# jackBonadies/Guided-Attention

Hardware: NVIDIA B200
Metric: guided_images_per_s (higher is better)
Workload: dtype f16

## Files before the change

guided_attention_b200/_cabi.py:

```python
from __future__ import annotations

import ctypes as C
import os
import threading

_HERE = os.path.dirname(os.path.abspath(__file__))
LIB_PATH = os.path.join(_HERE, "csrc", "libguidedattn.so")

GA_OK = 0
GA_F32, GA_F16, GA_BF16 = 0, 1, 2
GA_IMPL_AUTO, GA_IMPL_SIMT, GA_IMPL_TCGEN05, GA_IMPL_TCGEN05_SINGLE, GA_IMPL_TCGEN05_PIPE = 0, 1, 2, 3, 4
GA_TOKEN_COOR, GA_TOKEN_BOX, GA_TOKEN_KEYWORD = 0, 1, 2
GA_MAX_ACC_SLICES, GA_MAX_TOKENS, GA_MAX_BOXES, GA_MAX_CTX = 32, 24, 32, 128
(GA_STAT_MAX, GA_STAT_SUM, GA_STAT_COL, GA_STAT_ROW, GA_STAT_INSIDE, GA_STAT_OUTSIDE, GA_STAT_SCALED,
 GA_STAT_UNSCALED, GA_STAT_HINGE_IN, GA_STAT_HINGE_OUT, GA_STAT_NINSIDE, GA_STAT_CENTER, GA_STAT_RAW_SUM,
 GA_STAT_RAW_COL, GA_STAT_RAW_ROW) = range(15)
GA_STATS = 16
GA_ABI_VERSION = 7
GA_STEP_CTL_BYTES, GA_STEP_COUNTER_BASE = 256, 19
(GA_STEP_N_EVAL, GA_STEP_N_UPDATE, GA_STEP_N_CFG, GA_STEP_N_REFINE, GA_STEP_N_ROUNDS, GA_STEP_N_RENOISE) = range(6)


class GaToken(C.Structure):
    _fields_ = [("column", C.c_int32), ("kind", C.c_int32), ("box", C.c_int32), ("group", C.c_int32),
# ... 10 lines not shown

class GaScoreBias(C.Structure):
    _fields_ = [("mask", C.c_void_p), ("mask_stride_bh", C.c_int64), ("mask_stride_n", C.c_int64),
                ("pww_masks", C.c_void_p), ("pww_coef", C.c_void_p), ("pww_smax", C.c_void_p),
                ("pww_count", C.c_int32), ("pww_column", C.c_int32 * GA_MAX_TOKENS)]


class GaStepPrograms(C.Structure):
    _fields_ = [(n, C.c_void_p) for n in ("eval", "update", "cfg", "advance", "renoise", "refine_update")]


class GaStepParams(C.Structure):
    _fields_ = [("thr_call", C.c_double), ("thr_cfg", C.c_double), ("thr_last", C.c_double),
                ("has_thr_call", C.c_int32), ("has_thr_cfg", C.c_int32), ("has_thr_last", C.c_int32),
                ("check", C.c_int32), ("update_cond", C.c_int32), ("recurse_ok", C.c_int32),
                ("renoise_ok", C.c_int32), ("recurse_steps", C.c_int32), ("max_refine", C.c_int32),
                ("timestep", C.c_int64), ("step_size", C.c_float), ("ddim", C.c_float * 4),
                ("renoise", C.c_float * 2)]


_vp, _i, _f, _i64 = C.c_void_p, C.c_int, C.c_float, C.c_int64
_bias = C.POINTER(GaScoreBias)

PROTOTYPES = {
    "ga_version": (_i, []),
    "ga_last_error": (C.c_char_p, []),
    "ga_device_supported": (_i, [_i]),
    "ga_cross_attn_fwd": (_i, [_vp, _vp, _vp, _vp, _vp, _vp, _i, _i, _i, _i, _i, _f, _i, _i, _vp]),
    "ga_cross_attn_bwd": (_i, [_vp, _vp, _vp, _vp, _vp, _vp, _i64, _i, _vp, _vp, _vp, _i, _i, _i, _i, _i, _f, _i, _i,
                                _vp]),
    "ga_attn_probs": (_i, [_vp, _vp, _vp, _i, _i, _i, _i, _i, _f, _i, _vp]),
    "ga_cross_attn_smax": (_i, [_vp, _vp, _vp, _bias, _i, _i, _i, _i, _i, _f, _i, _vp]),
    "ga_cross_attn_fwd_ex": (_i, [_vp, _vp, _vp, _vp, _vp, _vp, _bias, _i, _i, _i, _i, _i, _f, _i, _i, _vp]),
    "ga_cross_attn_bwd_ex": (_i, [_vp, _vp, _vp, _vp, _vp, _vp, _i64, _i, _vp, _vp, _vp, _bias, _vp, _i, _i, _i, _i, _i,
                                   _f, _i, _i, _vp]),
    "ga_attn_probs_ex": (_i, [_vp, _vp, _vp, _bias, _i, _i, _i, _i, _i, _f, _i, _vp]),
    "ga_self_attn_fwd": (_i, [_vp, _vp, _vp, _vp, _vp, _i, _i, _i, _i, _f, _i, _vp]),
    "ga_self_attn_bwd": (_i, [_vp, _vp, _vp, _vp, _vp, _vp, _vp, _vp, _vp, _vp, _i, _i, _i, _i, _f, _i, _vp]),
    "ga_rasterize_boxes": (_i, [C.POINTER(C.c_double), _i, _i, C.c_double, _vp, _vp]),
    "ga_guidance_tail_fwd": (_i, [C.POINTER(_vp), C.POINTER(C.c_int32), _i, C.POINTER(GaTailParams), C.POINTER(GaToken),
                                  _vp, _vp, _vp, _vp, _vp, _vp, _vp, _vp, _vp]),
    "ga_guidance_tail_bwd": (_i, [C.POINTER(GaTailParams), C.POINTER(GaToken), _vp, _vp, _vp, _vp, _vp, _vp, _vp, _vp,
                                  _vp, _vp, _i, _vp]),
    "ga_step_driver_create": (_i, [C.POINTER(_vp), C.POINTER(GaStepPrograms), _vp, _vp, _vp, _vp, _vp, _vp, _vp, _vp,
                                   C.POINTER(GaToken), _i, _i, _i, _vp, _vp, _vp, _vp]),
    "ga_step_driver_run": (_i, [_vp, C.POINTER(GaStepParams), _vp]),
    "ga_step_driver_set_params": (_i, [_vp, C.POINTER(GaStepParams), _vp]),
    "ga_step_driver_destroy": (_i, [_vp]),
    "ga_smooth_fwd": (_i, [_vp, _vp, _i, _i, C.POINTER(C.c_float), _vp]),
    "ga_smooth_bwd": (_i, [_vp, _vp, _i, _i, C.POINTER(C.c_float), _vp]),
    "ga_box_loss_fwd": (_i, [_vp, _vp, _vp, _i, _i, _vp, _vp]),
    "ga_box_loss_bwd": (_i, [_vp, _vp, _vp, _i, _i, _vp, _vp, _vp]),
    "ga_group_norm_ws_bytes": (_i64, [_i, _i, _i, _i]),
    "ga_group_norm_fwd": (_i, [_vp, _vp, _i64, _vp, _vp, _vp, _vp, _vp, _i, _i, _i, _i, _f, _i, _i, _vp]),
    "ga_group_norm_bwd": (_i, [_vp, _vp, _i64, _vp, _vp, _vp, _vp, _vp, _vp, _i, _i, _i, _i, _i, _i, _vp]),
    "ga_add_bias_residual": (_i, [_vp, _vp, _vp, _vp, _i64, _i, _i, _vp]),
    "ga_layer_norm_fwd": (_i, [_vp, _vp, _vp, _vp, _vp, _vp, _i64, _i, _f, _i, _vp]),
    "ga_geglu_fwd": (_i, [_vp, _vp, _i64, _i, _i, _vp]),
    "ga_geglu_bwd": (_i, [_vp, _vp, _vp, _i64, _i, _i, _vp]),
}

_lib = None
_lock = threading.Lock()


class GuidedAttnLibraryError(RuntimeError):
    pass


def load(path: str = None) -> C.CDLL:
    global _lib
    with _lock:
        if _lib is not None and path is None:
            return _lib
        p = path or os.environ.get("GA_LIB_PATH", LIB_PATH)
        if not os.path.isfile(p):
            raise GuidedAttnLibraryError(
                f"{p} not found: build it with `python -c 'import __graft_entry__ as g; g.build()'` "
                "(nvcc, sm_100a).  The guidance path has no CPU or PyTorch fallback.")
        lib = C.CDLL(p)
        for name, (res, args) in PROTOTYPES.items():
            fn = getattr(lib, name)
            fn.restype, fn.argtypes = res, args
        if lib.ga_version() != GA_ABI_VERSION:
            raise GuidedAttnLibraryError(f"ABI mismatch: library {lib.ga_version()} vs binding {GA_ABI_VERSION}")
        if path is None:
            _lib = lib
        return lib


def check(rc: int, what: str):
    if rc != GA_OK:
        msg = load().ga_last_error().decode("utf-8", "replace")
        raise GuidedAttnLibraryError(f"{what} failed ({rc}): {msg}")
```

guided_attention_b200/csrc/unet_ops.cu:

```cuda
#include "ga_common.cuh"
#include <stdlib.h>

namespace ga {
namespace gn {

constexpr int kThreads = 256;

struct Params {
  const void* x;
  const void* dy;
  const void* gamma;
  const void* beta;
  const void* shift;
  int64_t shift_stride;
  void* out;
  float* stats;
  float* ws;
  int n, hw, c, groups, cpg;
  int cs;
  int vs;
  int pl;
  int chunk;
  int P;
  float eps;
};

template <typename T> __device__ __forceinline__ void unpack8(const uint4& w, float* f) {
  const float2 a = Word<T>::unpack(w.x), b = Word<T>::unpack(w.y), c = Word<T>::unpack(w.z), d = Word<T>::unpack(w.w);
  f[0] = a.x; f[1] = a.y; f[2] = b.x; f[3] = b.y; f[4] = c.x; f[5] = c.y; f[6] = d.x; f[7] = d.y;
}
template <typename T> __device__ __forceinline__ uint4 pack8(const float* f) {
  return make_uint4(Word<T>::pack(f[0], f[1]), Word<T>::pack(f[2], f[3]), Word<T>::pack(f[4], f[5]),
                    Word<T>::pack(f[6], f[7]));
}
__device__ __forceinline__ float sigmoidf_fast(float z) { return __fdividef(1.f, 1.f + __expf(-z)); }
__device__ __forceinline__ void pdl_wait() { asm volatile("griddepcontrol.wait;" ::: "memory"); }
__device__ __forceinline__ void pdl_launch_dependents() { asm volatile("griddepcontrol.launch_dependents;" ::: "memory"); }

struct Coord {
  int n, c0, pl, p0, p1;
  bool active;
  __device__ __forceinline__ void init(const Params& p) {
    const int tid = threadIdx.x;
    pl = tid / p.vs;
    const int v = tid - pl * p.vs;
    active = pl < p.pl;
    n = blockIdx.z;
    c0 = ((int)blockIdx.y * p.vs + v) * 8;
    p0 = (int)blockIdx.x * p.chunk;
    p1 = min(p0 + p.chunk, p.hw);
  }
};

template <typename T> __device__ __forceinline__ void load_shift(const Params& p, const Coord& t, float* sh) {
  if (p.shift != nullptr) {
    unpack8<T>(__ldg(reinterpret_cast<const uint4*>(reinterpret_cast<const T*>(p.shift) + (int64_t)t.n * p.shift_stride + t.c0)), sh);
  } else {
#pragma unroll
    for (int e = 0; e < 8; ++e) sh[e] = 0.f;
  }
}

__device__ __forceinline__ void group_partials(const Params& p, const Coord& t, const float* s, const float* q,
                                               float4* part, float& S, float& Q, int& g_out, bool& owner) {
  const int g0 = t.c0 / p.cpg;
  const int k = min(8, (g0 + 1) * p.cpg - t.c0);
  float sA = 0.f, qA = 0.f, sB = 0.f, qB = 0.f;
#pragma unroll
  for (int e = 0; e < 8; ++e) {
    if (e < k) { sA += s[e]; qA += q[e]; } else { sB += s[e]; qB += q[e]; }
  }
  part[threadIdx.x] = t.active ? make_float4(sA, qA, sB, qB) : make_float4(0.f, 0.f, 0.f, 0.f);
  __syncthreads();
  const int gps = p.groups / p.cs;
  const int sub = gps * 8 <= kThreads ? 8 : 1;
  const int gl = (int)threadIdx.x / sub, j = (int)threadIdx.x - gl * sub;
  const bool live = gl < gps;
  const int slice_c0 = (int)blockIdx.y * p.vs * 8;
  const int g = (int)blockIdx.y * gps + gl;
  S = 0.f; Q = 0.f;
  if (live) {
    const int v_lo = (g * p.cpg - slice_c0) >> 3, v_hi = ((g + 1) * p.cpg - 1 - slice_c0) >> 3;
    for (int l = j; l < p.pl; l += sub)
      for (int v = v_lo; v <= v_hi; ++v) {
        const float4 w = part[l * p.vs + v];
        if (slice_c0 + v * 8 >= g * p.cpg) { S += w.x; Q += w.y; } else { S += w.z; Q += w.w; }
      }
  }
  if (sub == 8) {
#pragma unroll
    for (int off = 4; off > 0; off >>= 1) {
      S += __shfl_down_sync(0xffffffffu, S, off, 8);
      Q += __shfl_down_sync(0xffffffffu, Q, off, 8);
    }
  }
  owner = live && j == 0;
  g_out = g;
}

constexpr int kMaxChunks = 128;
constexpr int kMaxSliceGroups = 32;
constexpr int kMergeLoads = 16;

__device__ __forceinline__ int merge_tpg(int gps) {
  int tpg = 8;
  while (tpg < 32 && tpg * 2 * gps <= kThreads) tpg *= 2;
  return tpg;
}

__device__ __forceinline__ void merge_stats(const Params& p, float2* sst) {
  pdl_wait();
  const int gps = p.groups / p.cs, n = blockIdx.z;
  const int tpg = merge_tpg(gps);
  const int gl = (int)threadIdx.x / tpg, j = (int)threadIdx.x - gl * tpg;
  const bool live = gl < gps;
  const int g = (int)blockIdx.y * gps + gl;
  float2 w[kMergeLoads];
#pragma unroll
  for (int i = 0; i < kMergeLoads; ++i) {
    const int ch = j + tpg * i;
    w[i] = (live && ch < p.P) ? __ldg(reinterpret_cast<const float2*>(p.ws) + ((int64_t)n * p.P + ch) * p.groups + g)
                              : make_float2(0.f, 0.f);
  }
  float cnt = 0.f, mean = 0.f, m2 = 0.f;
#pragma unroll
  for (int i = 0; i < kMergeLoads; ++i) {
    const int ch = j + tpg * i;
    if (live && ch < p.P) {
      const float cb = (float)((min((ch + 1) * p.chunk, p.hw) - ch * p.chunk) * p.cpg);
      const float tot = cnt + cb, delta = w[i].x - mean, f = __fdividef(cb, tot);
      mean = fmaf(delta, f, mean);
      m2 += w[i].y + delta * delta * cnt * f;
      cnt = tot;
    }
  }
#pragma unroll
  for (int off = 16; off > 0; off >>= 1) {
    if (off < tpg) {
      const float cb = __shfl_down_sync(0xffffffffu, cnt, off, 32);
      const float mb = __shfl_down_sync(0xffffffffu, mean, off, 32);
      const float qb = __shfl_down_sync(0xffffffffu, m2, off, 32);
      if (cb > 0.f && j + off < tpg) {
        const float tot = cnt + cb, delta = mb - mean, f = __fdividef(cb, tot);
        mean = fmaf(delta, f, mean);
        m2 += qb + delta * delta * cnt * f;
        cnt = tot;
// ... 184 lines not shown
template <typename T, bool kSilu>
__global__ void __launch_bounds__(kThreads) gn_bwd_apply_kernel(const Params p) {
  __shared__ float2 scf[kMaxSliceGroups];
  Coord t;
  t.init(p);
  merge_sums(p, scf);
  if (!t.active) return;
  float a[8], b[8], gr[8], r[8], mr[8], k1[8], k2[8];
  {
    float gm[8], bt[8];
    const int g_first = (int)blockIdx.y * (p.groups / p.cs);
    unpack8<T>(__ldg(reinterpret_cast<const uint4*>(reinterpret_cast<const T*>(p.gamma) + t.c0)), gm);
    unpack8<T>(__ldg(reinterpret_cast<const uint4*>(reinterpret_cast<const T*>(p.beta) + t.c0)), bt);
    float sh[8];
    load_shift<T>(p, t, sh);
#pragma unroll
    for (int e = 0; e < 8; ++e) {
      const int g = (t.c0 + e) / p.cpg;
      const float2 st = __ldg(reinterpret_cast<const float2*>(p.stats) + t.n * p.groups + g);
      const float2 cf = scf[g - g_first];
      const float mu = st.x - sh[e];
      r[e] = st.y;
      mr[e] = mu * st.y;
      a[e] = st.y * gm[e];
      b[e] = fmaf(-mu, a[e], bt[e]);
      gr[e] = gm[e] * st.y;
      k1[e] = cf.x * st.y;
      k2[e] = cf.y * st.y;
    }
  }
  const int64_t base = ((int64_t)t.n * p.hw) * p.c + t.c0;
  const uint4* xp = reinterpret_cast<const uint4*>(reinterpret_cast<const T*>(p.x) + base);
  const uint4* gp = reinterpret_cast<const uint4*>(reinterpret_cast<const T*>(p.dy) + base);
  uint4* op = reinterpret_cast<uint4*>(reinterpret_cast<T*>(p.out) + base);
  const int64_t stride = (int64_t)p.c / 8;
#pragma unroll 2
  for (int px = t.p0 + t.pl; px < t.p1; px += p.pl) {
    float f[8], d[8];
    unpack8<T>(__ldg(xp + px * stride), f);
    unpack8<T>(__ldg(gp + px * stride), d);
#pragma unroll
    for (int e = 0; e < 8; ++e) {
      float dz = d[e];
      if (kSilu) {
        const float z = fmaf(f[e], a[e], b[e]);
        const float sg = sigmoidf_fast(z);
        dz *= sg * fmaf(z, 1.f - sg, 1.f);
      }
      const float xh = fmaf(f[e], r[e], -mr[e]);
      f[e] = fmaf(dz, gr[e], -k1[e]) - xh * k2[e];
    }
    op[px * stride] = pack8<T>(f);
  }
}

static bool plan(Params& p, int n, int hw, int c, int groups) {
  if (n < 1 || hw < 1 || c < 8 || groups < 1 || c % groups != 0 || c % 8 != 0) return false;
  if ((int64_t)n * groups > (1 << 20)) return false;
  p.n = n; p.hw = hw; p.c = c; p.groups = groups; p.cpg = c / groups;
  const int V = c / 8;
  int cs = (V + kThreads - 1) / kThreads;
  while (cs <= groups && (groups % cs != 0 || V % cs != 0 || ((V / cs) * 8) % p.cpg != 0 || V / cs > kThreads)) ++cs;
  if (cs > groups) return false;
  p.cs = cs;
  p.vs = V / cs;
  p.pl = kThreads / p.vs;
  for (int v = 0; v < V; ++v)
    if ((v * 8 + 7) / p.cpg - (v * 8) / p.cpg > 1) return false;
  int chunk = (hw + 127) / 128;
  if (chunk < p.pl) chunk = p.pl;
  if (chunk > hw) chunk = hw;
  p.chunk = chunk;
  p.P = (hw + chunk - 1) / chunk;
  if (p.P > kMaxChunks || groups / cs > kMaxSliceGroups || n > 65535 || cs > 65535) return false;
  return true;
}

int64_t ws_bytes(int n, int hw, int c, int groups) {
  Params p;
  if (!plan(p, n, hw, c, groups)) return -1;
  return (int64_t)n * p.P * groups * 2 * (int64_t)sizeof(float);
}

static bool use_pdl() {
  static int v = -1;
  if (v < 0) {
    const char* e = getenv("GA_GN_PDL");
    v = (e != nullptr && e[0] == '0') ? 0 : 1;
  }
  return v == 1;
}

template <typename K>
static void launch_second(K kernel, const dim3& grid, const Params& p, cudaStream_t st) {
  cudaLaunchConfig_t cfg = {};
  cfg.gridDim = grid;
  cfg.blockDim = dim3(kThreads);
  cfg.dynamicSmemBytes = 0;
  cfg.stream = st;
  cudaLaunchAttribute attr[1];
  attr[0].id = cudaLaunchAttributeProgrammaticStreamSerialization;
  attr[0].val.programmaticStreamSerializationAllowed = 1;
  cfg.attrs = attr;
  cfg.numAttrs = use_pdl() ? 1 : 0;
  cudaLaunchKernelEx(&cfg, kernel, p);
}

template <typename T>
static void launch_fwd(const Params& p, bool silu, cudaStream_t st) {
  const dim3 grid(p.P, p.cs, p.n);
  gn_stats_kernel<T><<<grid, kThreads, 0, st>>>(p);
  if (silu) launch_second(gn_apply_kernel<T, true>, grid, p, st);
  else launch_second(gn_apply_kernel<T, false>, grid, p, st);
}
template <typename T>
static void launch_bwd(const Params& p, bool silu, cudaStream_t st) {
  const dim3 grid(p.P, p.cs, p.n);
  if (silu) {
    gn_bwd_sums_kernel<T, true><<<grid, kThreads, 0, st>>>(p);
    launch_second(gn_bwd_apply_kernel<T, true>, grid, p, st);
  } else {
    gn_bwd_sums_kernel<T, false><<<grid, kThreads, 0, st>>>(p);
    launch_second(gn_bwd_apply_kernel<T, false>, grid, p, st);
  }
}

int fwd(const void* x, const void* shift, int64_t shift_stride, const void* gamma, const void* beta, void* y, float* stats, float* ws, int n,
        int hw, int c, int groups, float eps, int silu, int dtype, cudaStream_t st) {
  Params p;
  if (!plan(p, n, hw, c, groups))
    return fail(GA_ERR_UNSUPPORTED, "group norm: shape n=%d hw=%d c=%d groups=%d is not supported", n, hw, c, groups);
  p.x = x; p.shift = shift; p.shift_stride = shift_stride; p.dy = nullptr; p.gamma = gamma; p.beta = beta; p.out = y; p.stats = stats; p.ws = ws;
  p.eps = eps;
  if (dtype == GA_F16) launch_fwd<__half>(p, silu != 0, st);
  else launch_fwd<__nv_bfloat16>(p, silu != 0, st);
  return check_launch("group_norm_fwd");
}

int bwd(const void* x, const void* shift, int64_t shift_stride, const void* dy, const void* gamma, const void* beta, const float* stats,
        void* dx, float* ws, int n, int hw, int c, int groups, int silu, int dtype, cudaStream_t st) {
  Params p;
  if (!plan(p, n, hw, c, groups))
    return fail(GA_ERR_UNSUPPORTED, "group norm: shape n=%d hw=%d c=%d groups=%d is not supported", n, hw, c, groups);
  p.x = x; p.shift = shift; p.shift_stride = shift_stride; p.dy = dy; p.gamma = gamma; p.beta = beta; p.out = dx; p.stats = const_cast<float*>(stats); p.ws = ws;
  p.eps = 0.f;
  if (dtype == GA_F16) launch_bwd<__half>(p, silu != 0, st);
  else launch_bwd<__nv_bfloat16>(p, silu != 0, st);
  return check_launch("group_norm_bwd");
}

template <typename T>
__global__ void __launch_bounds__(kThreads) add_bias_residual_kernel(const uint4* __restrict__ a, const uint4* __restrict__ b,
                                                                     const uint4* __restrict__ bias, uint4* __restrict__ out,
                                                                     int64_t n_vec, int vec_per_pixel) {
  for (int64_t i = (int64_t)blockIdx.x * kThreads + threadIdx.x; i < n_vec; i += (int64_t)gridDim.x * kThreads) {
    float fa[8], fb[8], fc[8];
    unpack8<T>(__ldg(a + i), fa);
    unpack8<T>(__ldg(bias + (int)(i % vec_per_pixel)), fc);
    if (b != nullptr) {
      unpack8<T>(__ldg(b + i), fb);
#pragma unroll
      for (int e = 0; e < 8; ++e) fa[e] += fb[e];
    }
#pragma unroll
    for (int e = 0; e < 8; ++e) fa[e] += fc[e];
    out[i] = pack8<T>(fa);
  }
}

int add_bias_residual(const void* a, const void* b, const void* bias, void* out, int64_t n_pixels, int c, int dtype,
                      cudaStream_t st) {
  const int64_t n_vec = n_pixels * (c / 8);
  if (n_vec == 0) return GA_OK;
  int64_t blocks = (n_vec + kThreads - 1) / kThreads;
  if (blocks > 148 * 8) blocks = 148 * 8;
  const uint4 *pa = static_cast<const uint4*>(a), *pb = static_cast<const uint4*>(b), *pc = static_cast<const uint4*>(bias);
  if (dtype == GA_F16)
    add_bias_residual_kernel<__half><<<(int)blocks, kThreads, 0, st>>>(pa, pb, pc, static_cast<uint4*>(out), n_vec, c / 8);
  else
    add_bias_residual_kernel<__nv_bfloat16><<<(int)blocks, kThreads, 0, st>>>(pa, pb, pc, static_cast<uint4*>(out), n_vec,
                                                                             c / 8);
  return check_launch("add_bias_residual");
}

__device__ __forceinline__ float gelu_f(float g) { return 0.5f * g * (1.f + erff(g * 0.70710678118654752f)); }
__device__ __forceinline__ float gelu_grad_f(float g) {
  return 0.5f * (1.f + erff(g * 0.70710678118654752f)) + g * 0.3989422804014327f * __expf(-0.5f * g * g);
}

template <typename T>
__global__ void __launch_bounds__(kThreads) geglu_fwd_kernel(const uint4* __restrict__ p, uint4* __restrict__ out,
                                                             int64_t n_vec, int vec_per_row) {
  for (int64_t i = (int64_t)blockIdx.x * kThreads + threadIdx.x; i < n_vec; i += (int64_t)gridDim.x * kThreads) {
    const int64_t r = i / vec_per_row;
    const int v = (int)(i - r * vec_per_row);
    float h[8], g[8];
    unpack8<T>(__ldg(p + r * 2 * vec_per_row + v), h);
    unpack8<T>(__ldg(p + r * 2 * vec_per_row + vec_per_row + v), g);
#pragma unroll
    for (int e = 0; e < 8; ++e) h[e] *= gelu_f(g[e]);
    out[i] = pack8<T>(h);
// ... 116 lines not shown
  GA_CHECK_ARG(x && gamma && beta && y && mean && rstd, "NULL operand");
  GA_CHECK_ARG(dtype == GA_F16 || dtype == GA_BF16, "layer norm: 16-bit activations only (dtype %d)", dtype);
  GA_CHECK_ARG(rows >= 0 && rows < ((int64_t)1 << 34) && channels >= 8 && channels % 8 == 0 &&
                   channels <= 32 * 8 * gn::kLnMaxVec,
               "layer norm: channels %d must be a multiple of 8 in [8, %d]", channels, 32 * 8 * gn::kLnMaxVec);
  GA_CHECK_ALIGN(x, 16, "x");
  GA_CHECK_ALIGN(y, 16, "y");
  GA_CHECK_ALIGN(gamma, 16, "gamma");
  GA_CHECK_ALIGN(beta, 16, "beta");
  return gn::layer_norm_fwd(x, gamma, beta, y, mean, rstd, rows, channels, eps, dtype, static_cast<cudaStream_t>(stream));
}

static int check_geglu_args(const void* p, const void* out, int64_t rows, int inner, int dtype) {
  GA_CHECK_ARG(p && out, "NULL operand");
  GA_CHECK_ARG(dtype == GA_F16 || dtype == GA_BF16, "geglu: 16-bit activations only (dtype %d)", dtype);
  GA_CHECK_ARG(rows >= 0 && inner >= 8 && inner % 8 == 0, "geglu: inner width %d must be a multiple of 8", inner);
  GA_CHECK_ALIGN(p, 16, "proj");
  GA_CHECK_ALIGN(out, 16, "output");
  return GA_OK;
}

extern "C" int ga_geglu_fwd(const void* proj, void* out, int64_t rows, int inner, int dtype, ga_stream_t stream) {
  int rc = check_geglu_args(proj, out, rows, inner, dtype);
  if (rc != GA_OK) return rc;
  return gn::geglu(proj, nullptr, out, rows, inner, dtype, false, static_cast<cudaStream_t>(stream));
}

extern "C" int ga_geglu_bwd(const void* proj, const void* d_out, void* d_proj, int64_t rows, int inner, int dtype,
                            ga_stream_t stream) {
  int rc = check_geglu_args(proj, d_proj, rows, inner, dtype);
  if (rc != GA_OK) return rc;
  GA_CHECK_ARG(d_out != nullptr, "NULL operand");
  GA_CHECK_ALIGN(d_out, 16, "d_out");
  return gn::geglu(proj, d_out, d_proj, rows, inner, dtype, true, static_cast<cudaStream_t>(stream));
}

extern "C" int ga_add_bias_residual(const void* a, const void* b, const void* bias, void* out, int64_t n_pixels,
                                    int channels, int dtype, ga_stream_t stream) {
  GA_CHECK_ARG(a && bias && out, "NULL operand");
  GA_CHECK_ARG(dtype == GA_F16 || dtype == GA_BF16, "add_bias_residual: 16-bit activations only (dtype %d)", dtype);
  GA_CHECK_ARG(n_pixels >= 0 && channels >= 8 && channels % 8 == 0, "add_bias_residual: channels %d must be a multiple of 8",
               channels);
  GA_CHECK_ALIGN(a, 16, "a");
  GA_CHECK_ALIGN(out, 16, "out");
  GA_CHECK_ALIGN(bias, 16, "bias");
  if (b != nullptr) GA_CHECK_ALIGN(b, 16, "b");
  return gn::add_bias_residual(a, b, bias, out, n_pixels, channels, dtype, static_cast<cudaStream_t>(stream));
}

extern "C" int64_t ga_group_norm_ws_bytes(int n, int hw, int channels, int groups) {
  return gn::ws_bytes(n, hw, channels, groups);
}

static int check_gn_args(const void* x, const void* gamma, const void* beta, const void* out, const void* stats,
                         const void* ws, int dtype) {
  GA_CHECK_ARG(x && gamma && beta && out && stats && ws, "NULL operand");
  GA_CHECK_ARG(dtype == GA_F16 || dtype == GA_BF16, "group norm: 16-bit activations only (dtype %d)", dtype);
  GA_CHECK_ALIGN(x, 16, "x");
  GA_CHECK_ALIGN(out, 16, "output");
  GA_CHECK_ALIGN(gamma, 16, "gamma");
  GA_CHECK_ALIGN(beta, 16, "beta");
  GA_CHECK_ALIGN(stats, 8, "stats");
  GA_CHECK_ALIGN(ws, 8, "ws");
  return GA_OK;
}

extern "C" int ga_group_norm_fwd(const void* x, const void* shift, int64_t shift_stride, const void* gamma, const void* beta, void* y,
                                 float* stats, float* ws, int n, int hw, int channels, int groups, float eps, int silu,
                                 int dtype, ga_stream_t stream) {
  int rc = check_gn_args(x, gamma, beta, y, stats, ws, dtype);
  if (rc != GA_OK) return rc;
  if (shift != nullptr) {
    GA_CHECK_ALIGN(shift, 16, "shift");
    GA_CHECK_ARG(shift_stride >= channels && shift_stride % 8 == 0, "shift_stride %lld must be a multiple of 8 >= channels",
                 (long long)shift_stride);
  }
  return gn::fwd(x, shift, shift_stride, gamma, beta, y, stats, ws, n, hw, channels, groups, eps, silu, dtype,
                 static_cast<cudaStream_t>(stream));
}

extern "C" int ga_group_norm_bwd(const void* x, const void* shift, int64_t shift_stride, const void* d_y, const void* gamma, const void* beta,
                                 const float* stats, void* d_x, float* ws, int n, int hw, int channels, int groups,
                                 int silu, int dtype, ga_stream_t stream) {
  int rc = check_gn_args(x, gamma, beta, d_x, stats, ws, dtype);
  if (rc != GA_OK) return rc;
  GA_CHECK_ARG(d_y != nullptr, "NULL operand");
  GA_CHECK_ALIGN(d_y, 16, "d_y");
  if (shift != nullptr) {
    GA_CHECK_ALIGN(shift, 16, "shift");
    GA_CHECK_ARG(shift_stride >= channels && shift_stride % 8 == 0, "shift_stride %lld must be a multiple of 8 >= channels",
                 (long long)shift_stride);
  }
  return gn::bwd(x, shift, shift_stride, d_y, gamma, beta, stats, d_x, ws, n, hw, channels, groups, silu, dtype,
                 static_cast<cudaStream_t>(stream));
}
```

guided_attention_b200/ops.py:

```python
from __future__ import annotations

import ctypes as C
import math
import os
from dataclasses import dataclass, field
from typing import List, Optional, Sequence

import numpy as np
import torch

from . import _cabi as abi

launch_counts = {}


def _count(name, n=1):
    launch_counts[name] = launch_counts.get(name, 0) + n


def total_launches() -> int:
    return sum(launch_counts.values())


def reset_launch_counts():
# ... 280 lines not shown
        ctx.save_for_backward(q.contiguous(), k.contiguous(), v.contiguous(), o, lse)
        ctx.meta = (heads, float(scale))
        return o

    @staticmethod
    def backward(ctx, d_o):
        q, k, v, o, lse = ctx.saved_tensors
        heads, scale = ctx.meta
        lib = abi.load()
        B, N, Cdim = q.shape
        d = Cdim // heads
        d_o = d_o.contiguous()
        d_q, d_k, d_v = torch.empty_like(q), torch.empty_like(k), torch.empty_like(v)
        dvec = torch.empty((B, heads, N), dtype=torch.float32, device=q.device)
        with torch.cuda.device(q.device), _span("self_attn_bwd", (B, heads, N, d, str(q.dtype)),
                                                self_attn_flops(B, heads, N, d, "bwd"), q.device):
            abi.check(lib.ga_self_attn_bwd(_ptr(q), _ptr(k), _ptr(v), _ptr(o), _ptr(lse), _ptr(d_o), _ptr(d_q),
                                           _ptr(d_k), _ptr(d_v), _ptr(dvec), B, heads, N, d, scale,
                                           _DTYPES[q.dtype], _stream(q)), "ga_self_attn_bwd")
        _count("self_attn_bwd", 2)
        return d_q, d_k, d_v, None, None


def self_attention(q, k, v, heads: int, scale: float):
    return _SelfAttnFn.apply(q, k, v, heads, scale)


def self_attention_supported(dtype, head_dim: int) -> bool:
    return dtype in (torch.float16, torch.bfloat16) and head_dim % 8 == 0 and 8 <= head_dim <= 160


def attention_probs(q, k, heads: int, scale: float, bias=None):
    _need_cuda(q, k)
    lib = abi.load()
    q, k = q.contiguous(), k.contiguous()
    B, N, Cdim = q.shape
    T = k.shape[1]
    p = torch.empty((B * heads, N, T), dtype=q.dtype, device=q.device)
    with torch.cuda.device(q.device):
        if bias is not None:
            if bias.has_pww and bias.smax is None:
                score_max(q, k, heads, scale, bias)
            sb = bias.struct(B, heads, N, T, q.device)
            abi.check(lib.ga_attn_probs_ex(_ptr(q), _ptr(k), _ptr(p), C.byref(sb), B, heads, N, T, Cdim // heads,
                                           float(scale), _DTYPES[q.dtype], _stream(q)), "ga_attn_probs_ex")
        else:
            abi.check(lib.ga_attn_probs(_ptr(q), _ptr(k), _ptr(p), B, heads, N, T, Cdim // heads, float(scale),
                                        _DTYPES[q.dtype], _stream(q)), "ga_attn_probs")
    _count("attn_probs")
    return p


_gn_plan_cache = {}


def group_norm_ws_bytes(n: int, hw: int, c: int, groups: int) -> int:
    key = (n, hw, c, groups)
    if key not in _gn_plan_cache:
        _gn_plan_cache[key] = int(abi.load().ga_group_norm_ws_bytes(n, hw, c, groups))
    return _gn_plan_cache[key]


def group_norm_supported(x: torch.Tensor, weight, bias, groups: int) -> bool:
    if not (x.is_cuda and x.dim() == 4 and x.dtype in (torch.float16, torch.bfloat16)):
        return False
    if weight is None or bias is None or weight.requires_grad or bias.requires_grad:
        return False
    n, c, h, w = x.shape
    return group_norm_ws_bytes(n, h * w, c, groups) >= 0


class _GroupNormFn(torch.autograd.Function):
    @staticmethod
    def forward(ctx, x, weight, bias, shift, groups: int, eps: float, silu: bool):
        _need_cuda(x, weight, bias, shift)
        lib = abi.load()
        x = x.contiguous(memory_format=torch.channels_last)
        n, c, h, w = x.shape
        if weight.dtype != x.dtype:
            weight, bias = weight.to(x.dtype), bias.to(x.dtype)
        weight, bias = weight.contiguous(), bias.contiguous()
        if shift is not None:
            shift = shift.to(x.dtype).reshape(n, c)
            if shift.stride(1) != 1 or shift.stride(0) % 8 != 0 or shift.stride(0) < c or shift.data_ptr() % 16 != 0:
                shift = shift.contiguous()
        y = torch.empty_like(x)
        stats = torch.empty(n, groups, 2, dtype=torch.float32, device=x.device)
        ws = torch.empty(max(group_norm_ws_bytes(n, h * w, c, groups), 8) // 4, dtype=torch.float32, device=x.device)
        nbytes = 3 * x.numel() * x.element_size()
        with torch.cuda.device(x.device), _span("group_norm_fwd", (n, h * w, c, groups, int(silu)), nbytes, x.device):
            abi.check(lib.ga_group_norm_fwd(_ptr(x), _ptr(shift), shift.stride(0) if shift is not None else 0,
                                            _ptr(weight), _ptr(bias), _ptr(y), _ptr(stats),
                                            _ptr(ws), n, h * w, c, groups, float(eps), int(silu), _DTYPES[x.dtype],
                                            _stream(x)), "ga_group_norm_fwd")
        _count("group_norm_fwd", 2)
        ctx.save_for_backward(x, weight, bias, stats, shift)
        ctx.meta = (groups, bool(silu))
        return y

    @staticmethod
    def backward(ctx, d_y):
        x, weight, bias, stats, shift = ctx.saved_tensors
        groups, silu = ctx.meta
        lib = abi.load()
        n, c, h, w = x.shape
        d_y = d_y.contiguous(memory_format=torch.channels_last)
        d_x = torch.empty_like(x)
        ws = torch.empty(max(group_norm_ws_bytes(n, h * w, c, groups), 8) // 4, dtype=torch.float32, device=x.device)
        nbytes = 5 * x.numel() * x.element_size()
        with torch.cuda.device(x.device), _span("group_norm_bwd", (n, h * w, c, groups, int(silu)), nbytes, x.device):
            abi.check(lib.ga_group_norm_bwd(_ptr(x), _ptr(shift), shift.stride(0) if shift is not None else 0,
                                            _ptr(d_y), _ptr(weight), _ptr(bias), _ptr(stats),
                                            _ptr(d_x), _ptr(ws), n, h * w, c, groups, int(silu), _DTYPES[x.dtype],
                                            _stream(x)), "ga_group_norm_bwd")
        _count("group_norm_bwd", 2)
        return d_x, None, None, None, None, None, None


def group_norm(x, weight, bias, groups: int, eps: float = 1e-5, silu: bool = False, shift=None):
    if shift is not None and shift.requires_grad:
        raise ValueError("group_norm: `shift` must not require a gradient (only x is differentiated)")
    return _GroupNormFn.apply(x, weight, bias, shift, int(groups), float(eps), bool(silu))


class _AddBiasResidualFn(torch.autograd.Function):
    @staticmethod
    def forward(ctx, a, bias, b):
        _need_cuda(a, bias, b)
        lib = abi.load()
        a = a.contiguous(memory_format=torch.channels_last)
        n, c, h, w = a.shape
        if b is not None:
            b = b.contiguous(memory_format=torch.channels_last)
        bias = bias.to(a.dtype).contiguous()
        out = torch.empty_like(a)
        nbytes = (3 if b is not None else 2) * a.numel() * a.element_size()
        with torch.cuda.device(a.device), _span("add_bias_residual", (n, h * w, c, int(b is not None)), nbytes, a.device):
            abi.check(lib.ga_add_bias_residual(_ptr(a), _ptr(b), _ptr(bias), _ptr(out), n * h * w, c, _DTYPES[a.dtype],
                                               _stream(a)), "ga_add_bias_residual")
        _count("add_bias_residual")
        ctx.has_b = b is not None
        return out

    @staticmethod
    def backward(ctx, g):
        return g, None, (g if ctx.has_b else None)


def add_bias_residual(a, bias, b=None):
    if bias.requires_grad:
        raise ValueError("add_bias_residual: `bias` must not require a gradient")
    return _AddBiasResidualFn.apply(a, bias, b)


class _GegluFn(torch.autograd.Function):
    @staticmethod
    def forward(ctx, proj):
        _need_cuda(proj)
        lib = abi.load()
        proj = proj.contiguous()
        inner = proj.shape[-1] // 2
        rows = proj.numel() // (2 * inner)
        out = torch.empty(proj.shape[:-1] + (inner,), dtype=proj.dtype, device=proj.device)
        with torch.cuda.device(proj.device), _span("geglu_fwd", (rows, inner), 3 * rows * inner * proj.element_size(),
                                                   proj.device):
            abi.check(lib.ga_geglu_fwd(_ptr(proj), _ptr(out), rows, inner, _DTYPES[proj.dtype], _stream(proj)),
                      "ga_geglu_fwd")
        _count("geglu_fwd")
# ... 269 lines not shown
```

include/guided_attn.h:

```cpp
#ifndef GUIDED_ATTN_H_
#define GUIDED_ATTN_H_

#include <stdint.h>

#ifdef __cplusplus
extern "C" {
#endif

#define GA_ABI_VERSION 7

typedef void* ga_stream_t;

enum ga_status { GA_OK = 0, GA_ERR_BAD_ARG = -1, GA_ERR_UNSUPPORTED = -2, GA_ERR_ALIGNMENT = -3, GA_ERR_CUDA = -4 };
enum ga_dtype { GA_F32 = 0, GA_F16 = 1, GA_BF16 = 2 };
enum ga_impl { GA_IMPL_AUTO = 0, GA_IMPL_SIMT = 1, GA_IMPL_TCGEN05 = 2, GA_IMPL_TCGEN05_SINGLE = 3,
               GA_IMPL_TCGEN05_PIPE = 4 };
enum ga_token_kind { GA_TOKEN_COOR = 0, GA_TOKEN_BOX = 1, GA_TOKEN_KEYWORD = 2 };

#define GA_MAX_ACC_SLICES 32
#define GA_MAX_TOKENS 24
#define GA_MAX_BOXES 32
#define GA_MAX_CTX 128

enum ga_stat {
// ... 97 lines not shown
                         const ga_tail_params_t* params_host, const ga_token_t* tokens_host, const uint8_t* masks,
                         const float* weights, float* attn_text, float* smoothed, float* stats, int32_t* argmax,
                         float* total, uint32_t* ticket, ga_stream_t stream);

int ga_guidance_tail_bwd(const ga_tail_params_t* params_host, const ga_token_t* tokens_host, const uint8_t* masks,
                         const float* weights, const float* attn_text, const float* smoothed, const float* stats,
                         const int32_t* argmax, const float* g_total, const float* g_stats, const float* g_attn_text,
                         float* d_abar, int d_abar_row_stride, ga_stream_t stream);

#define GA_STEP_CTL_BYTES 256
typedef struct ga_step_programs {
  void *eval, *update, *cfg, *advance, *renoise;
  void* refine_update;
} ga_step_programs_t;

typedef struct ga_step_params {
  double thr_call;
  double thr_cfg;
  double thr_last;
  int32_t has_thr_call, has_thr_cfg, has_thr_last;
  int32_t check;
  int32_t update_cond;
  int32_t recurse_ok;
  int32_t renoise_ok;
  int32_t recurse_steps;
  int32_t max_refine;
  int64_t timestep;
  float step_size;
  float ddim[4];
  float renoise[2];
} ga_step_params_t;

int ga_step_driver_create(void** driver_out, const ga_step_programs_t* programs, void* ctl_dev,
                          const float* stats_eval, const float* stats_update, const float* custom_eval,
                          const float* custom_update, const float* stats_refine, const float* custom_refine,
                          float* refine_first_dev, const ga_token_t* tokens_host, int n_tokens, int n_groups,
                          int avg_within, int64_t* t_dev, float* step_dev, float* ddim_dev, float* renoise_dev);
int ga_step_driver_run(void* driver, const ga_step_params_t* params_host, ga_stream_t stream);
int ga_step_driver_set_params(void* driver, const ga_step_params_t* params_host, ga_stream_t stream);
int ga_step_driver_destroy(void* driver);
enum ga_step_counter { GA_STEP_N_EVAL = 0, GA_STEP_N_UPDATE = 1, GA_STEP_N_CFG = 2, GA_STEP_N_REFINE = 3,
                       GA_STEP_N_ROUNDS = 4, GA_STEP_N_RENOISE = 5 };
#define GA_STEP_COUNTER_BASE 19

int ga_smooth_fwd(const float* maps, float* out, int n_maps, int res, const float* w1d_host, ga_stream_t stream);
int ga_smooth_bwd(const float* g_out, float* g_maps, int n_maps, int res, const float* w1d_host, ga_stream_t stream);

int ga_box_loss_fwd(const float* p, const uint8_t* mask, const float* weights, int res, int strict, float* out2,
                    ga_stream_t stream);
int ga_box_loss_bwd(const float* p, const uint8_t* mask, const float* weights, int res, int strict,
                    const float* g_out2, float* g_p, ga_stream_t stream);

int64_t ga_group_norm_ws_bytes(int n, int hw, int channels, int groups);
int ga_group_norm_fwd(const void* x, const void* shift, int64_t shift_stride, const void* gamma, const void* beta,
                      void* y, float* stats, float* ws, int n, int hw, int channels, int groups, float eps, int silu,
                      int dtype, ga_stream_t stream);
int ga_group_norm_bwd(const void* x, const void* shift, int64_t shift_stride, const void* d_y, const void* gamma,
                      const void* beta, const float* stats, void* d_x, float* ws, int n, int hw, int channels, int groups,
                      int silu, int dtype, ga_stream_t stream);
int ga_add_bias_residual(const void* a, const void* b, const void* bias, void* out, int64_t n_pixels, int channels,
                         int dtype, ga_stream_t stream);

int ga_geglu_fwd(const void* proj, void* out, int64_t rows, int inner, int dtype, ga_stream_t stream);
int ga_geglu_bwd(const void* proj, const void* d_out, void* d_proj, int64_t rows, int inner, int dtype,
                 ga_stream_t stream);

int ga_layer_norm_fwd(const void* x, const void* gamma, const void* beta, void* y, float* mean, float* rstd,
                      int64_t rows, int channels, float eps, int dtype, ga_stream_t stream);

#ifdef __cplusplus
}
#endif
#endif
```

Baseline: 0.7726.

## Fuse group norm into single cluster kernel with DSMEM stats exchange for low-res layers

Adds single-launch fused forward and backward group-norm kernels for wide-channel, small-spatial layers (c>=1920, 64<hw<=256). Inputs are staged in shared memory, and per-group partial statistics are combined across CTAs of a thread-block cluster through distributed shared memory instead of a global workspace and a second launch. This removes one kernel launch and the re-read of x (and dy in backward) from global memory. The cost is large dynamic shared-memory use, which can limit occupancy, plus cluster barriers. group_partials also gains a configurable subgroup width.

```diff
diff --git a/guided_attention_b200/_cabi.py b/guided_attention_b200/_cabi.py
--- a/guided_attention_b200/_cabi.py
+++ b/guided_attention_b200/_cabi.py
@@ -86,6 +86,7 @@
     "ga_box_loss_fwd": (_i, [_vp, _vp, _vp, _i, _i, _vp, _vp]),
     "ga_box_loss_bwd": (_i, [_vp, _vp, _vp, _i, _i, _vp, _vp, _vp]),
     "ga_group_norm_ws_bytes": (_i64, [_i, _i, _i, _i]),
+    "ga_group_norm_launches": (_i, [_i, _i, _i, _i]),
     "ga_group_norm_fwd": (_i, [_vp, _vp, _i64, _vp, _vp, _vp, _vp, _vp, _i, _i, _i, _i, _f, _i, _i, _vp]),
     "ga_group_norm_bwd": (_i, [_vp, _vp, _i64, _vp, _vp, _vp, _vp, _vp, _vp, _i, _i, _i, _i, _i, _i, _vp]),
     "ga_add_bias_residual": (_i, [_vp, _vp, _vp, _vp, _i64, _i, _i, _vp]),
diff --git a/guided_attention_b200/csrc/unet_ops.cu b/guided_attention_b200/csrc/unet_ops.cu
--- a/guided_attention_b200/csrc/unet_ops.cu
+++ b/guided_attention_b200/csrc/unet_ops.cu
@@ -61,6 +61,7 @@
   }
 }
 
+template <int kSub = 8>
 __device__ __forceinline__ void group_partials(const Params& p, const Coord& t, const float* s, const float* q,
                                                float4* part, float& S, float& Q, int& g_out, bool& owner) {
   const int g0 = t.c0 / p.cpg;
@@ -73,7 +74,8 @@
   part[threadIdx.x] = t.active ? make_float4(sA, qA, sB, qB) : make_float4(0.f, 0.f, 0.f, 0.f);
   __syncthreads();
   const int gps = p.groups / p.cs;
-  const int sub = gps * 8 <= kThreads ? 8 : 1;
+  int sub = kSub;
+  while (sub > 1 && gps * sub > kThreads) sub >>= 1;
   const int gl = (int)threadIdx.x / sub, j = (int)threadIdx.x - gl * sub;
   const bool live = gl < gps;
   const int slice_c0 = (int)blockIdx.y * p.vs * 8;
@@ -87,11 +89,11 @@
         if (slice_c0 + v * 8 >= g * p.cpg) { S += w.x; Q += w.y; } else { S += w.z; Q += w.w; }
       }
   }
-  if (sub == 8) {
-#pragma unroll
-    for (int off = 4; off > 0; off >>= 1) {
-      S += __shfl_down_sync(0xffffffffu, S, off, 8);
-      Q += __shfl_down_sync(0xffffffffu, Q, off, 8);
+#pragma unroll
+  for (int off = kSub / 2; off > 0; off >>= 1) {
+    if (off < sub) {
+      S += __shfl_down_sync(0xffffffffu, S, off, sub);
+      Q += __shfl_down_sync(0xffffffffu, Q, off, sub);
     }
   }
   owner = live && j == 0;
@@ -382,6 +384,239 @@
     }
     op[px * stride] = pack8<T>(f);
   }
+}
+
+constexpr int kMaxCluster = 8;
+constexpr int kFusedSub = 32;
+
+__device__ __forceinline__ void cluster_arrive() { asm volatile("barrier.cluster.arrive.release.aligned;" ::: "memory"); }
+__device__ __forceinline__ void cluster_wait() { asm volatile("barrier.cluster.wait.acquire.aligned;" ::: "memory"); }
+__device__ __forceinline__ void cluster_arrive_relaxed() {
+  asm volatile("barrier.cluster.arrive.relaxed.aligned;" ::: "memory");
+}
+__device__ __forceinline__ float2 ld_cluster(const float2* v, int rank) {
+  uint32_t a = (uint32_t)__cvta_generic_to_shared(v), r;
+  asm volatile("mapa.shared::cluster.u32 %0, %1, %2;" : "=r"(r) : "r"(a), "r"(rank));
+  float2 w;
+  asm volatile("ld.shared::cluster.v2.f32 {%0, %1}, [%2];" : "=f"(w.x), "=f"(w.y) : "r"(r) : "memory");
+  return w;
+}
+__device__ __forceinline__ float rank_count(const Params& p, int rank) {
+  return (float)(max(min((rank + 1) * p.chunk, p.hw) - rank * p.chunk, 0) * p.cpg);
+}
+
+template <typename T, bool kSilu>
+__global__ void __launch_bounds__(kThreads) gn_fused_fwd_kernel(const Params p) {
+  extern __shared__ uint4 stage[];
+  __shared__ float4 part[kThreads];
+  __shared__ float2 xchg[kMaxSliceGroups];
+  __shared__ float2 sst[kMaxSliceGroups];
+  Coord t;
+  t.init(p);
+  const int gps = p.groups / p.cs, g_first = (int)blockIdx.y * gps;
+  const int64_t base = ((int64_t)t.n * p.hw) * p.c + t.c0;
+  const int64_t stride = (int64_t)p.c / 8;
+  float sh[8], s[8], q[8];
+#pragma unroll
+  for (int e = 0; e < 8; ++e) { s[e] = 0.f; q[e] = 0.f; sh[e] = 0.f; }
+  if (t.active) {
+    load_shift<T>(p, t, sh);
+    const uint4* xp = reinterpret_cast<const uint4*>(reinterpret_cast<const T*>(p.x) + base);
+    int i = 0;
+#pragma unroll 4
+    for (int px = t.p0 + t.pl; px < t.p1; px += p.pl, ++i) {
+      const uint4 w = __ldg(xp + px * stride);
+      stage[i * kThreads + threadIdx.x] = w;
+      float f[8];
+      unpack8<T>(w, f);
+#pragma unroll
+      for (int e = 0; e < 8; ++e) s[e] += f[e] + sh[e];
+    }
+  }
+  float S, Q;
+  int g;
+  bool owner;
+  const float cnt = rank_count(p, blockIdx.x);
+  group_partials<kFusedSub>(p, t, s, q, part, S, Q, g, owner);
+  if (owner) sst[g - g_first] = make_float2(cnt > 0.f ? S / cnt : 0.f, 0.f);
+  __syncthreads();
+  if (t.active) {
+    float m[8];
+#pragma unroll
+    for (int e = 0; e < 8; ++e) m[e] = sst[(t.c0 + e) / p.cpg - g_first].x - sh[e];
+    int i = 0;
+    for (int px = t.p0 + t.pl; px < t.p1; px += p.pl, ++i) {
+      float f[8];
+      unpack8<T>(stage[i * kThreads + threadIdx.x], f);
+#pragma unroll
+      for (int e = 0; e < 8; ++e) {
+        const float d = f[e] - m[e];
+        q[e] = fmaf(d, d, q[e]);
+      }
+    }
+  }
+  group_partials<kFusedSub>(p, t, s, q, part, S, Q, g, owner);
+  if (owner) xchg[g - g_first] = make_float2(sst[g - g_first].x, Q);
+  cluster_arrive();
+  cluster_wait();
+  if (threadIdx.x < gps) {
+    float2 w[kMaxCluster];
+#pragma unroll
+    for (int r = 0; r < kMaxCluster; ++r) w[r] = r < (int)gridDim.x ? ld_cluster(&xchg[threadIdx.x], r) : make_float2(0.f, 0.f);
+    float n_a = 0.f, mean = 0.f, m2 = 0.f;
+#pragma unroll
+    for (int r = 0; r < kMaxCluster; ++r) {
+      const float n_b = r < (int)gridDim.x ? rank_count(p, r) : 0.f;
+      if (n_b > 0.f) {
+        const float tot = n_a + n_b, delta = w[r].x - mean, f = n_b / tot;
+        mean = fmaf(delta, f, mean);
+        m2 += w[r].y + delta * delta * n_a * f;
+        n_a = tot;
+      }
+    }
+    const float2 st = make_float2(mean, rsqrtf(m2 / n_a + p.eps));
+    sst[threadIdx.x] = st;
+    if (blockIdx.x == 0) reinterpret_cast<float2*>(p.stats)[t.n * p.groups + g_first + threadIdx.x] = st;
+  }
+  cluster_arrive_relaxed();
+  __syncthreads();
+  if (t.active) {
+    float a[8], b[8];
+    {
+      float gm[8], bt[8];
+      unpack8<T>(__ldg(reinterpret_cast<const uint4*>(reinterpret_cast<const T*>(p.gamma) + t.c0)), gm);
+      unpack8<T>(__ldg(reinterpret_cast<const uint4*>(reinterpret_cast<const T*>(p.beta) + t.c0)), bt);
+#pragma unroll
+      for (int e = 0; e < 8; ++e) {
+        const float2 st = sst[(t.c0 + e) / p.cpg - g_first];
+        a[e] = st.y * gm[e];
+        b[e] = fmaf(sh[e] - st.x, a[e], bt[e]);
+      }
+    }
+    uint4* yp = reinterpret_cast<uint4*>(reinterpret_cast<T*>(p.out) + base);
+    int i = 0;
+#pragma unroll 4
+    for (int px = t.p0 + t.pl; px < t.p1; px += p.pl, ++i) {
+      float f[8];
+      unpack8<T>(stage[i * kThreads + threadIdx.x], f);
+#pragma unroll
+      for (int e = 0; e < 8; ++e) {
+        const float z = fmaf(f[e], a[e], b[e]);
+        f[e] = kSilu ? z * sigmoidf_fast(z) : z;
+      }
+      yp[px * stride] = pack8<T>(f);
+    }
+  }
+  cluster_wait();
+}
+
+template <typename T, bool kSilu>
+__global__ void __launch_bounds__(kThreads) gn_fused_bwd_kernel(const Params p) {
+  extern __shared__ uint4 stage[];
+  __shared__ float4 part[kThreads];
+  __shared__ float2 xchg[kMaxSliceGroups];
+  __shared__ float2 scf[kMaxSliceGroups];
+  Coord t;
+  t.init(p);
+  const int gps = p.groups / p.cs, g_first = (int)blockIdx.y * gps;
+  const int iters = (p.chunk + p.pl - 1) / p.pl;
+  const int64_t base = ((int64_t)t.n * p.hw) * p.c + t.c0;
+  const int64_t stride = (int64_t)p.c / 8;
+  float a[8], b[8], gm[8], r[8], mr[8], s[8], q[8];
+#pragma unroll
+  for (int e = 0; e < 8; ++e) { s[e] = 0.f; q[e] = 0.f; }
+  if (t.active) {
+    {
+      float bt[8], sh[8];
+      unpack8<T>(__ldg(reinterpret_cast<const uint4*>(reinterpret_cast<const T*>(p.gamma) + t.c0)), gm);
+      unpack8<T>(__ldg(reinterpret_cast<const uint4*>(reinterpret_cast<const T*>(p.beta) + t.c0)), bt);
+      load_shift<T>(p, t, sh);
+#pragma unroll
+      for (int e = 0; e < 8; ++e) {
+        const float2 st = __ldg(reinterpret_cast<const float2*>(p.stats) + t.n * p.groups + (t.c0 + e) / p.cpg);
+        const float mu = st.x - sh[e];
+        r[e] = st.y;
+        mr[e] = mu * st.y;
+        a[e] = st.y * gm[e];
+        b[e] = fmaf(-mu, a[e], bt[e]);
+      }
+    }
+    const uint4* xp = reinterpret_cast<const uint4*>(reinterpret_cast<const T*>(p.x) + base);
+    const uint4* gp = reinterpret_cast<const uint4*>(reinterpret_cast<const T*>(p.dy) + base);
+    int i = 0;
+#pragma unroll 2
+    for (int px = t.p0 + t.pl; px < t.p1; px += p.pl, ++i) {
+      const uint4 wx = __ldg(xp + px * stride), wd = __ldg(gp + px * stride);
+      stage[i * kThreads + threadIdx.x] = wx;
+      stage[(iters + i) * kThreads + threadIdx.x] = wd;
+      float f[8], d[8];
+      unpack8<T>(wx, f);
+      unpack8<T>(wd, d);
+#pragma unroll
+      for (int e = 0; e < 8; ++e) {
+        float dz = d[e];
+        if (kSilu) {
+          const float z = fmaf(f[e], a[e], b[e]);
+          const float sg = sigmoidf_fast(z);
+          dz *= sg * fmaf(z, 1.f - sg, 1.f);
+        }
+        const float dxh = dz * gm[e];
+        const float xh = fmaf(f[e], r[e], -mr[e]);
+        s[e] += dxh;
+        q[e] = fmaf(dxh, xh, q[e]);
+      }
+    }
+  }
+  float S, Q;
+  int g;
+  bool owner;
+  group_partials<kFusedSub>(p, t, s, q, part, S, Q, g, owner);
+  if (owner) xchg[g - g_first] = make_float2(S, Q);
+  cluster_arrive();
+  cluster_wait();
+  if (threadIdx.x < gps) {
+    float2 w[kMaxCluster];
+#pragma unroll
+    for (int k = 0; k < kMaxCluster; ++k) w[k] = k < (int)gridDim.x ? ld_cluster(&xchg[threadIdx.x], k) : make_float2(0.f, 0.f);
+    float s1 = 0.f, s2 = 0.f;
+#pragma unroll
+    for (int k = 0; k < kMaxCluster; ++k) { s1 += w[k].x; s2 += w[k].y; }
+    const float inv_m = 1.f / ((float)p.hw * (float)p.cpg);
+    scf[threadIdx.x] = make_float2(s1 * inv_m, s2 * inv_m);
+  }
+  cluster_arrive_relaxed();
+  __syncthreads();
+  if (t.active) {
+    float gr[8], k1[8], k2[8];
+#pragma unroll
+    for (int e = 0; e < 8; ++e) {
+      const float2 cf = scf[(t.c0 + e) / p.cpg - g_first];
+      gr[e] = gm[e] * r[e];
+      k1[e] = cf.x * r[e];
+      k2[e] = cf.y * r[e];
+    }
+    uint4* op = reinterpret_cast<uint4*>(reinterpret_cast<T*>(p.out) + base);
+    int i = 0;
+#pragma unroll 2
+    for (int px = t.p0 + t.pl; px < t.p1; px += p.pl, ++i) {
+      float f[8], d[8];
+      unpack8<T>(stage[i * kThreads + threadIdx.x], f);
+      unpack8<T>(stage[(iters + i) * kThreads + threadIdx.x], d);
+#pragma unroll
+      for (int e = 0; e < 8; ++e) {
+        float dz = d[e];
+        if (kSilu) {
+          const float z = fmaf(f[e], a[e], b[e]);
+          const float sg = sigmoidf_fast(z);
+          dz *= sg * fmaf(z, 1.f - sg, 1.f);
+        }
+        const float xh = fmaf(f[e], r[e], -mr[e]);
+        f[e] = fmaf(dz, gr[e], -k1[e]) - xh * k2[e];
+      }
+      op[px * stride] = pack8<T>(f);
+    }
+  }
+  cluster_wait();
 }
 
 static bool plan(Params& p, int n, int hw, int c, int groups) {
@@ -412,6 +647,33 @@
   return (int64_t)n * p.P * groups * 2 * (int64_t)sizeof(float);
 }
 
+constexpr int kFusedCtasPerSample = 128;
+constexpr int kMaxStageBytes = 96 * 1024;
+
+static bool plan_fused(Params& p, int n, int hw, int c, int groups) {
+  if (c < 1920 || hw <= 64 || hw > 256 || !plan(p, n, hw, c, groups)) return false;
+  const int V = c / 8;
+  int cs = 0, P = 0;
+  for (int k = p.cs; k <= groups; ++k) {
+    if (groups % k != 0 || V % k != 0 || ((V / k) * 8) % p.cpg != 0) continue;
+    cs = k;
+    P = min(kMaxCluster, (hw + kThreads / (V / k) - 1) / (kThreads / (V / k)));
+    if (cs * P >= kFusedCtasPerSample) break;
+  }
+  p.cs = cs;
+  p.vs = V / cs;
+  p.pl = kThreads / p.vs;
+  p.chunk = (hw + P - 1) / P;
+  p.P = (hw + p.chunk - 1) / p.chunk;
+  return (int64_t)((p.chunk + p.pl - 1) / p.pl) * kThreads * sizeof(uint4) <= kMaxStageBytes;
+}
+
+int launches(int n, int hw, int c, int groups) {
+  Params p;
+  if (plan_fused(p, n, hw, c, groups)) return 1;
+  return plan(p, n, hw, c, groups) ? 2 : -1;
+}
+
 static bool use_pdl() {
   static int v = -1;
   if (v < 0) {
@@ -455,28 +717,82 @@
   }
 }
 
+static int raise_fused_limits() {
+  static bool raised[64] = {};
+  int dev = 0;
+  cudaGetDevice(&dev);
+  if (dev < 0 || dev >= 64 || raised[dev]) return GA_OK;
+  const void* kernels[] = {
+      (const void*)gn_fused_fwd_kernel<__half, true>, (const void*)gn_fused_fwd_kernel<__half, false>,
+      (const void*)gn_fused_fwd_kernel<__nv_bfloat16, true>, (const void*)gn_fused_fwd_kernel<__nv_bfloat16, false>,
+      (const void*)gn_fused_bwd_kernel<__half, true>, (const void*)gn_fused_bwd_kernel<__half, false>,
+      (const void*)gn_fused_bwd_kernel<__nv_bfloat16, true>, (const void*)gn_fused_bwd_kernel<__nv_bfloat16, false>};
+  for (const void* k : kernels) {
+    cudaError_t e = cudaFuncSetAttribute(k, cudaFuncAttributeMaxDynamicSharedMemorySize, 2 * kMaxStageBytes);
+    if (e != cudaSuccess) return fail(GA_ERR_CUDA, "group norm: cudaFuncSetAttribute: %s", cudaGetErrorString(e));
+  }
+  raised[dev] = true;
+  return GA_OK;
+}
+
+template <typename K>
+static int launch_fused(K kernel, const Params& p, int tensors, cudaStream_t st) {
+  const int rc = raise_fused_limits();
+  if (rc != GA_OK) return rc;
+  const int smem = tensors * ((p.chunk + p.pl - 1) / p.pl) * kThreads * (int)sizeof(uint4);
+  cudaLaunchConfig_t cfg = {};
+  cfg.gridDim = dim3(p.P, p.cs, p.n);
+  cfg.blockDim = dim3(kThreads);
+  cfg.dynamicSmemBytes = smem;
+  cfg.stream = st;
+  cudaLaunchAttribute attr[1];
+  attr[0].id = cudaLaunchAttributeClusterDimension;
+  attr[0].val.clusterDim.x = p.P;
+  attr[0].val.clusterDim.y = 1;
+  attr[0].val.clusterDim.z = 1;
+  cfg.attrs = attr;
+  cfg.numAttrs = 1;
+  cudaLaunchKernelEx(&cfg, kernel, p);
+  return GA_OK;
+}
+
+template <typename T>
+static int launch_fused_fwd(const Params& p, bool silu, cudaStream_t st) {
+  return silu ? launch_fused(gn_fused_fwd_kernel<T, true>, p, 1, st) : launch_fused(gn_fused_fwd_kernel<T, false>, p, 1, st);
+}
+template <typename T>
+static int launch_fused_bwd(const Params& p, bool silu, cudaStream_t st) {
+  return silu ? launch_fused(gn_fused_bwd_kernel<T, true>, p, 2, st) : launch_fused(gn_fused_bwd_kernel<T, false>, p, 2, st);
+}
+
 int fwd(const void* x, const void* shift, int64_t shift_stride, const void* gamma, const void* beta, void* y, float* stats, float* ws, int n,
         int hw, int c, int groups, float eps, int silu, int dtype, cudaStream_t st) {
   Params p;
-  if (!plan(p, n, hw, c, groups))
+  const bool one = plan_fused(p, n, hw, c, groups);
+  if (!one && !plan(p, n, hw, c, groups))
     return fail(GA_ERR_UNSUPPORTED, "group norm: shape n=%d hw=%d c=%d groups=%d is not supported", n, hw, c, groups);
   p.x = x; p.shift = shift; p.shift_stride = shift_stride; p.dy = nullptr; p.gamma = gamma; p.beta = beta; p.out = y; p.stats = stats; p.ws = ws;
   p.eps = eps;
-  if (dtype == GA_F16) launch_fwd<__half>(p, silu != 0, st);
+  int rc = GA_OK;
+  if (one) rc = dtype == GA_F16 ? launch_fused_fwd<__half>(p, silu != 0, st) : launch_fused_fwd<__nv_bfloat16>(p, silu != 0, st);
+  else if (dtype == GA_F16) launch_fwd<__half>(p, silu != 0, st);
   else launch_fwd<__nv_bfloat16>(p, silu != 0, st);
-  return check_launch("group_norm_fwd");
+  return rc != GA_OK ? rc : check_launch("group_norm_fwd");
 }
 
 int bwd(const void* x, const void* shift, int64_t shift_stride, const void* dy, const void* gamma, const void* beta, const float* stats,
         void* dx, float* ws, int n, int hw, int c, int groups, int silu, int dtype, cudaStream_t st) {
   Params p;
-  if (!plan(p, n, hw, c, groups))
+  const bool one = plan_fused(p, n, hw, c, groups);
+  if (!one && !plan(p, n, hw, c, groups))
     return fail(GA_ERR_UNSUPPORTED, "group norm: shape n=%d hw=%d c=%d groups=%d is not supported", n, hw, c, groups);
   p.x = x; p.shift = shift; p.shift_stride = shift_stride; p.dy = dy; p.gamma = gamma; p.beta = beta; p.out = dx; p.stats = const_cast<float*>(stats); p.ws = ws;
   p.eps = 0.f;
-  if (dtype == GA_F16) launch_bwd<__half>(p, silu != 0, st);
+  int rc = GA_OK;
+  if (one) rc = dtype == GA_F16 ? launch_fused_bwd<__half>(p, silu != 0, st) : launch_fused_bwd<__nv_bfloat16>(p, silu != 0, st);
+  else if (dtype == GA_F16) launch_bwd<__half>(p, silu != 0, st);
   else launch_bwd<__nv_bfloat16>(p, silu != 0, st);
-  return check_launch("group_norm_bwd");
+  return rc != GA_OK ? rc : check_launch("group_norm_bwd");
 }
 
 template <typename T>
@@ -699,6 +1015,10 @@
   return gn::ws_bytes(n, hw, channels, groups);
 }
 
+extern "C" int ga_group_norm_launches(int n, int hw, int channels, int groups) {
+  return gn::launches(n, hw, channels, groups);
+}
+
 static int check_gn_args(const void* x, const void* gamma, const void* beta, const void* out, const void* stats,
                          const void* ws, int dtype) {
   GA_CHECK_ARG(x && gamma && beta && out && stats && ws, "NULL operand");
diff --git a/guided_attention_b200/ops.py b/guided_attention_b200/ops.py
--- a/guided_attention_b200/ops.py
+++ b/guided_attention_b200/ops.py
@@ -356,6 +356,7 @@
 
 
 _gn_plan_cache = {}
+_gn_launch_cache = {}
 
 
 def group_norm_ws_bytes(n: int, hw: int, c: int, groups: int) -> int:
@@ -363,6 +364,13 @@
     if key not in _gn_plan_cache:
         _gn_plan_cache[key] = int(abi.load().ga_group_norm_ws_bytes(n, hw, c, groups))
     return _gn_plan_cache[key]
+
+
+def group_norm_launches(n: int, hw: int, c: int, groups: int) -> int:
+    key = (n, hw, c, groups)
+    if key not in _gn_launch_cache:
+        _gn_launch_cache[key] = int(abi.load().ga_group_norm_launches(n, hw, c, groups))
+    return _gn_launch_cache[key]
 
 
 def group_norm_supported(x: torch.Tensor, weight, bias, groups: int) -> bool:
@@ -391,13 +399,14 @@
         y = torch.empty_like(x)
         stats = torch.empty(n, groups, 2, dtype=torch.float32, device=x.device)
         ws = torch.empty(max(group_norm_ws_bytes(n, h * w, c, groups), 8) // 4, dtype=torch.float32, device=x.device)
-        nbytes = 3 * x.numel() * x.element_size()
+        launches = group_norm_launches(n, h * w, c, groups)
+        nbytes = (1 + launches) * x.numel() * x.element_size()
         with torch.cuda.device(x.device), _span("group_norm_fwd", (n, h * w, c, groups, int(silu)), nbytes, x.device):
             abi.check(lib.ga_group_norm_fwd(_ptr(x), _ptr(shift), shift.stride(0) if shift is not None else 0,
                                             _ptr(weight), _ptr(bias), _ptr(y), _ptr(stats),
                                             _ptr(ws), n, h * w, c, groups, float(eps), int(silu), _DTYPES[x.dtype],
                                             _stream(x)), "ga_group_norm_fwd")
-        _count("group_norm_fwd", 2)
+        _count("group_norm_fwd", launches)
         ctx.save_for_backward(x, weight, bias, stats, shift)
         ctx.meta = (groups, bool(silu))
         return y
@@ -411,13 +420,14 @@
         d_y = d_y.contiguous(memory_format=torch.channels_last)
         d_x = torch.empty_like(x)
         ws = torch.empty(max(group_norm_ws_bytes(n, h * w, c, groups), 8) // 4, dtype=torch.float32, device=x.device)
-        nbytes = 5 * x.numel() * x.element_size()
+        launches = group_norm_launches(n, h * w, c, groups)
+        nbytes = (1 + 2 * launches) * x.numel() * x.element_size()
         with torch.cuda.device(x.device), _span("group_norm_bwd", (n, h * w, c, groups, int(silu)), nbytes, x.device):
             abi.check(lib.ga_group_norm_bwd(_ptr(x), _ptr(shift), shift.stride(0) if shift is not None else 0,
                                             _ptr(d_y), _ptr(weight), _ptr(bias), _ptr(stats),
                                             _ptr(d_x), _ptr(ws), n, h * w, c, groups, int(silu), _DTYPES[x.dtype],
                                             _stream(x)), "ga_group_norm_bwd")
-        _count("group_norm_bwd", 2)
+        _count("group_norm_bwd", launches)
         return d_x, None, None, None, None, None, None
 
 
diff --git a/include/guided_attn.h b/include/guided_attn.h
--- a/include/guided_attn.h
+++ b/include/guided_attn.h
@@ -173,6 +173,7 @@
                     const float* g_out2, float* g_p, ga_stream_t stream);
 
 int64_t ga_group_norm_ws_bytes(int n, int hw, int channels, int groups);
+int ga_group_norm_launches(int n, int hw, int channels, int groups);
 int ga_group_norm_fwd(const void* x, const void* shift, int64_t shift_stride, const void* gamma, const void* beta,
                       void* y, float* stats, float* ws, int n, int hw, int channels, int groups, float eps, int silu,
                       int dtype, ga_stream_t stream);
```

Result: no change. 0.7727 (median of 6 runs) (+0.0%).
